# nicolapiccinelli/libmpc

Hardware: AMD Instinct MI355X
Metric: MPC solves/sec (whole node) + p50 solve latency, quadrotor LMPC N=20 batch=4096 (higher is better)
Workload: dtype f64; 1 GPU; quadrotor_ex.cpp LMPC nx=12 nu=4 ny=12 ph=ch=20, batch 4096 per GPU, SplitMix64 x0/u0/yref (SURVEY 8d), maximum_iteration=250; parallelism=single GPU, rccl_ranks=0, streams=1

## Files before the change

### libmpc_amd/csrc/lmpc_fast.hip

```cpp
#include "lmpc_kernel_common.hpp"
#include <cstddef>
#include <cstdlib>

namespace mpcx {

namespace {

#ifndef MPCX_FAST_PF_MAXCAP
#define MPCX_FAST_PF_MAXCAP 12
#endif
#ifndef MPCX_FAST_RB
#define MPCX_FAST_RB 4
#endif
#ifndef MPCX_FAST_PF
#define MPCX_FAST_PF 4
#endif
constexpr int kFastCap = 16;
#ifndef MPCX_FAST_ADD_THETA_LATE
#define MPCX_FAST_ADD_THETA_LATE 0.02
#endif
#ifndef MPCX_FAST_SAFE_AFTER
#define MPCX_FAST_SAFE_AFTER 12
#endif

template <int CTRL>
__device__ __forceinline__ double dpp_mov_d(double v)
{
    int lo = __double2loint(v), hi = __double2hiint(v);
    lo = __builtin_amdgcn_update_dpp(lo, lo, CTRL, 0xF, 0xF, false);
    hi = __builtin_amdgcn_update_dpp(hi, hi, CTRL, 0xF, 0xF, false);
    return __hiloint2double(hi, lo);
}
__device__ __forceinline__ double wave_max_dpp(double v)
{
    v = fmax(v, dpp_mov_d<0xB1>(v));
    v = fmax(v, dpp_mov_d<0x4E>(v));
    v = fmax(v, dpp_mov_d<0x141>(v));
    v = fmax(v, dpp_mov_d<0x140>(v));
    return fmax(fmax(readlane_d(v, 0), readlane_d(v, 16)), fmax(readlane_d(v, 32), readlane_d(v, 48)));
}

#ifdef MPCX_PROFILE_ROUNDS
#define MPCX_LAP(k) do { const long long now_ = (long long)__builtin_readcyclecounter(); pacc[k] += now_ - plast; plast = now_; } while (0)
#define MPCX_LAP_WAIT(k) do { __builtin_amdgcn_s_waitcnt(0); MPCX_LAP(k); } while (0)
#define MPCX_PROF_ARGS , long long (&pacc)[6], long long &plast
#define MPCX_PROF_PASS , pacc, plast
#else
#define MPCX_LAP(k) do {} while (0)
#define MPCX_LAP_WAIT(k) do {} while (0)
#define MPCX_PROF_ARGS
#define MPCX_PROF_PASS
#endif

template <int CAP, int NLO, int CPZ, int CPG>
__device__ __forceinline__ int ws_solve_reg(const gdp gY, const int ldy, const int ldz, const int na, const int lane_in,
                                            const int *wsidx, const double *wsb, const double *t0s, double *lam,
                                            const unsigned (&offz)[CPZ], const unsigned (&offg)[CPG],
                                            double (&wv)[2 * CPZ], double (&gw)[2 * CPG], double &lmax MPCX_PROF_ARGS)
{
    constexpr int PF = CAP > MPCX_FAST_PF_MAXCAP ? 0 : (CAP < MPCX_FAST_PF ? CAP : MPCX_FAST_PF);
    int lane = lane_in;
    asm volatile("" : "+v"(lane));
    const bool real = lane < na;
    const int li = real ? lane : 0;
    const int qi = wsidx[li];
    int qc[CAP];
#pragma unroll
    for (int c = 0; c < CAP; ++c) qc[c] = __builtin_amdgcn_readfirstlane(wsidx[(c < NLO || c < na) ? c : 0]);
    double Sr[CAP];
    const unsigned rowoff = (unsigned)(qi * ldy) * 8u;
    const char MPCX_GAS *const gYb = reinterpret_cast<const char MPCX_GAS *>(gY);
    auto y_at = [&](unsigned off) { return *reinterpret_cast<gdp>(gYb + off); };
    auto row_ld2 = [&](int q, unsigned off) { return *reinterpret_cast<const d2 MPCX_GAS *>(gYb + (unsigned)(q * ldy) * 8u + off); };
#pragma unroll
    for (int c = 0; c < CAP; ++c) Sr[c] = y_at(rowoff + (unsigned)qc[c] * 8u);
    const double dg = y_at(rowoff + (unsigned)qi * 8u);
    d2 pz[PF > 0 ? PF : 1][CPZ], pg[PF > 0 ? PF : 1][CPG];
#pragma unroll
    for (int u = 0; u < PF; ++u) {
#pragma unroll
        for (int c = 0; c < CPZ; ++c) pz[u][c] = row_ld2(qc[u], offz[c]);
#pragma unroll
        for (int c = 0; c < CPG; ++c) pg[u][c] = row_ld2(qc[u], offg[c]);
    }
    double y = real ? t0s[qi < ldz ? qi : qi - ldz + 128 * CPZ] - wsb[li] : 0.0;
    MPCX_LAP_WAIT(1);
    if (!real) {
#pragma unroll
        for (int c = 0; c < CAP; ++c) Sr[c] = 0.0;
    }
#pragma unroll
    for (int c = NLO; c < CAP; ++c) if (c >= na) Sr[c] = lane == c ? 1.0 : 0.0;
    const double pthr = 1e-11 * (real ? dg : 1.0);
    double mydinv = 1.0;
    unsigned long long dep = 0ull;
#pragma unroll
    for (int k = 0; k < CAP; ++k) {
        dep |= __ballot(!(Sr[k] > pthr)) & (1ull << k);
        const double rinv = pivot_rcp(readlane_d(Sr[k], k));
        double pj[CAP];
#pragma unroll
        for (int j = k + 1; j < CAP; ++j) pj[j] = readlane_d(Sr[j], k);
        const double py = readlane_d(y, k);
        if (lane == k) mydinv = rinv;
        else {
            const double m = Sr[k] * rinv;
#pragma unroll
            for (int j = k + 1; j < CAP; ++j) Sr[j] = fma(-m, pj[j], Sr[j]);
            y = fma(-m, py, y);
        }
    }
    MPCX_LAP(2);
    if (dep != 0ull) return (int)__builtin_ctzll(dep);
    y *= mydinv;
    if (real) lam[lane] = y;
#pragma unroll
    for (int c = 0; c < CPZ; ++c) {
        const double2 v = *reinterpret_cast<const double2 *>(t0s + 128 * c + 2 * lane);
        wv[2 * c] = v.x; wv[2 * c + 1] = v.y;
    }
#pragma unroll
    for (int c = 0; c < CPG; ++c) {
        const double2 v = *reinterpret_cast<const double2 *>(t0s + 128 * CPZ + 128 * c + 2 * lane);
        gw[2 * c] = v.x; gw[2 * c + 1] = v.y;
    }
    double lm = 0.0;
#pragma unroll
    for (int a = 0; a < PF; ++a) {
        const double la = readlane_d(y, a);
        lm = fmax(lm, fabs(la));
#pragma unroll
        for (int c = 0; c < CPZ; ++c) { wv[2 * c] = fma(-la, pz[a][c].x, wv[2 * c]); wv[2 * c + 1] = fma(-la, pz[a][c].y, wv[2 * c + 1]); }
#pragma unroll
        for (int c = 0; c < CPG; ++c) { gw[2 * c] = fma(-la, pg[a][c].x, gw[2 * c]); gw[2 * c + 1] = fma(-la, pg[a][c].y, gw[2 * c + 1]); }
    }
    if constexpr (CAP > PF) {
        constexpr int RB = CAP - PF < MPCX_FAST_RB ? CAP - PF : MPCX_FAST_RB;
        int again = 0;
        asm volatile("" : "+s"(again));
        const int *wsidx_again = wsidx + again;
#pragma unroll
        for (int a0 = PF; a0 < CAP; a0 += RB) {
            if (a0 < na) {
                d2 mz[RB][CPZ], mgv[RB][CPG];
#pragma unroll
                for (int u = 0; u < RB; ++u) {
                    const int cu = a0 + u < CAP ? a0 + u : 0;
                    const int q = __builtin_amdgcn_readfirstlane(wsidx_again[(cu < NLO || cu < na) ? cu : 0]);
#pragma unroll
                    for (int c = 0; c < CPZ; ++c) mz[u][c] = row_ld2(q, offz[c]);
#pragma unroll
                    for (int c = 0; c < CPG; ++c) mgv[u][c] = row_ld2(q, offg[c]);
                }
#pragma unroll
                for (int u = 0; u < RB; ++u) {
                    if (a0 + u < CAP) {
                        const double la = readlane_d(y, a0 + u < CAP ? a0 + u : 0);
                        lm = fmax(lm, fabs(la));
#pragma unroll
                        for (int c = 0; c < CPZ; ++c) { wv[2 * c] = fma(-la, mz[u][c].x, wv[2 * c]); wv[2 * c + 1] = fma(-la, mz[u][c].y, wv[2 * c + 1]); }
#pragma unroll
                        for (int c = 0; c < CPG; ++c) { gw[2 * c] = fma(-la, mgv[u][c].x, gw[2 * c]); gw[2 * c + 1] = fma(-la, mgv[u][c].y, gw[2 * c + 1]); }
                    }
                }
            }
        }
    }
    lmax = lm;
    return -1;
}

template <int CPZ, int CPG>
__device__ __forceinline__ void fast_init_pads(double *slice, const int ldz, const int ldg, const int lane)
{
    constexpr int ZP = 128 * CPZ, GPD = 128 * CPG;
    const double INF = __builtin_huge_val();
    double *t0s = slice, *gt0s = t0s + ZP, *lgs = gt0s + GPD, *ugs = lgs + GPD, *fs = ugs + GPD, *lam = fs + ZP + 2;
#pragma unroll
    for (int c = 0; c < CPZ; ++c) {
        const int e = 128 * c + 2 * lane;
        if (e >= ldz) { *reinterpret_cast<double2 *>(t0s + e) = make_double2(0.0, 0.0); *reinterpret_cast<double2 *>(fs + e) = make_double2(0.0, 0.0); }
    }
#pragma unroll
    for (int c = 0; c < CPG; ++c) {
        const int r = 128 * c + 2 * lane;
        if (r >= ldg) {
            *reinterpret_cast<double2 *>(gt0s + r) = make_double2(0.0, 0.0);
            *reinterpret_cast<double2 *>(lgs + r) = make_double2(-INF, -INF);
            *reinterpret_cast<double2 *>(ugs + r) = make_double2(INF, INF);
        }
    }
    if (lane == 0) { lam[kFastCap] = 0.0; lam[kFastCap + 1] = 0.0; }
}

template <int CPZ, int CPG> constexpr int fast_slice_fixed() { return 2 * 128 * CPZ + 3 * 128 * CPG + 2 + 2 * (kFastCap + 2) + (kFastCap + 2) / 2 + 1; }

constexpr int kCpFused = 3;
struct RecPtrs { double *f, *t0, *gt0, *lg, *ug, *tail; };
__device__ __forceinline__ void fused_record(const LmpcDev &M, const LmpcBatchDev &Bt, const int b, const int lane, double *stage,
                                             const RecPtrs &rp, const double *mf_lds)
{
    const int nx = M.nx, nu = M.nu, ny = M.ny, kin = M.kin;
    const int ldz = M.ldz, ldg = M.ldg, ldy = M.ldy, rowsF = M.rowsF;
    const int variant = Bt.fused - 1;
    for (int k = lane; k < kin; k += 64) {
        double v = 0.0;
        if (k < M.nxp) { if (k < nx) v = gl(Bt.x0)[(size_t)b * nx + k]; }
        else if (k < M.nxp + M.nup) { const int c = k - M.nxp; if (c < nu) v = gl(Bt.u0)[(size_t)b * nu + c]; }
        else if (k < M.ione) { const int c = k - M.nxp - M.nup; if (variant && c < ny) v = gl(Bt.yref)[(size_t)b * Bt.yref_bs + c]; }
        else if (k == M.ione) v = 1.0;
        stage[k] = v;
    }
    wave_sync();
    double acc[2 * kCpFused];
#pragma unroll
    for (int s = 0; s < 2 * kCpFused; ++s) acc[s] = 0.0;
    if (mf_lds) {
        int off[kCpFused];
#pragma unroll
        for (int c = 0; c < kCpFused; ++c) { const int e = 128 * c + 2 * lane; off[c] = e < rowsF ? e : 0; }
        for (int j = 0; j < kin; j += 4) {
            double2 m[4][kCpFused];
            double xj[4];
#pragma unroll
            for (int u = 0; u < 4; ++u) {
                const double *col = mf_lds + (size_t)(j + u) * rowsF;
#pragma unroll
                for (int c = 0; c < kCpFused; ++c) m[u][c] = *reinterpret_cast<const double2 *>(col + off[c]);
                xj[u] = stage[j + u];
            }
#pragma unroll
            for (int u = 0; u < 4; ++u) {
#pragma unroll
                for (int c = 0; c < kCpFused; ++c) {
                    acc[2 * c] = fma(m[u][c].x, xj[u], acc[2 * c]);
                    acc[2 * c + 1] = fma(m[u][c].y, xj[u], acc[2 * c + 1]);
                }
            }
        }
    } else {
        matvec_acc<kCpFused>(gl(variant ? M.MF1 : M.MF0), rowsF, rowsF, kin, stage, acc, lane);
    }
    const int r_goff = ldy, r_f = r_goff + ldg, r_s = r_f + ldz, r_q = r_s + M.nsp;
    double c0p = 0.0;
    bool bad = false;
#pragma unroll
    for (int c = 0; c < kCpFused; ++c) {
        const int e = 128 * c + 2 * lane;
        if (e >= rowsF) continue;
        const double a0 = acc[2 * c], a1 = acc[2 * c + 1];
        if (e < ldz) {
            *reinterpret_cast<double2 *>(rp.t0 + e) = make_double2(a0, a1);
        } else if (e < r_goff) {
            *reinterpret_cast<double2 *>(rp.gt0 + (e - ldz)) = make_double2(a0, a1);
        } else if (e < r_f) {
            const int r = e - r_goff;
            const d2 l0 = ld2(GP(lg0) + r), u0 = ld2(GP(ug0) + r);
            *reinterpret_cast<double2 *>(rp.lg + r) = make_double2(l0.x - a0, l0.y - a1);
            *reinterpret_cast<double2 *>(rp.ug + r) = make_double2(u0.x - a0, u0.y - a1);
        } else if (e < r_s) {
            *reinterpret_cast<double2 *>(rp.f + (e - r_f)) = make_double2(a0, a1);
        } else if (e < r_q) {
            const int r = e - r_s;
            if (r < M.ns) bad |= violates(a0, GP(slo)[r], GP(shi)[r], M.eps_abs, M.eps_rel);
            if (r + 1 < M.ns) bad |= violates(a1, GP(slo)[r + 1], GP(shi)[r + 1], M.eps_abs, M.eps_rel);
        } else {
            const int k = e - r_q;
            c0p = fma(0.5 * stage[k], a0, c0p);
            c0p = fma(0.5 * stage[k + 1], a1, c0p);
        }
    }
    c0p = wave_sum(c0p);
    const bool anybad = wave_any(bad);
    if (lane == 0) *reinterpret_cast<double2 *>(rp.tail) = make_double2(c0p, anybad ? 1.0 : 0.0);
    wave_sync();
}

struct GroupArgs { LmpcDev M; LmpcBatchDev Bt; double *wsbase; int variant; };
typedef const GroupArgs __attribute__((address_space(4))) *group_args_p;
static_assert(offsetof(GroupArgs, Bt) == sizeof(LmpcDev) && offsetof(GroupArgs, wsbase) == sizeof(LmpcDev) + sizeof(LmpcBatchDev), "GroupArgs mirrors lmpc_solve_group's parameter list");

template <int CPZ, int CPG, int SRC>
__device__ __forceinline__ void fast_finish(const LmpcDev &M, const LmpcBatchDev &Bt, const int b, const int lane, double *slice, const double *lwuw, gdw ws, double *outs,
                                            const bool infeasible, const bool solved, const bool fixed_violation,
                                            const double (&wv)[2 * CPZ], const int (&actb)[2 * CPZ], const int (&actg)[2 * CPG], const int (&posb)[2 * CPZ],
                                            const int (&posg)[2 * CPG], const double dtol_last, const int na_last, const int rounds_total,
                                            const long long ts0, const long long ts1, const long long ts2 MPCX_PROF_ARGS)
{
    constexpr int NZS = 2 * CPZ, NGS = 2 * CPG, ZP = 128 * CPZ, GPD = 128 * CPG;
    constexpr bool FUSED = SRC != 0;
    const int nx = M.nx, nu = M.nu, ny = M.ny, ndu = M.ndu, ph = M.ph;
    const int nz = M.nz, mg = M.mg, ldz = M.ldz, ldg = M.ldg, ldy = M.ldy;
    double *t0s = slice, *gt0s = t0s + ZP, *lgs = gt0s + GPD, *ugs = lgs + GPD, *fs = ugs + GPD, *tail = fs + ZP;
    double *lam = tail + 2, *wsb = lam + (kFastCap + 2);
    double *scratch = wsb + (kFastCap + 2) + (kFastCap + 2) / 2 + 1;
    const double *lws = lwuw, *uws = lwuw + ZP;
    const double c0 = tail[0], flag0 = tail[1];
    long long ts3 = 0;
    auto stamp = [&](long long &t) { if (Bt.dbg_cycles) t = (long long)__builtin_readcyclecounter(); };

    if (!infeasible && !solved) {
        if constexpr (FUSED) {
#pragma unroll
            for (int c = 0; c < CPZ; ++c) {
                const int e = 128 * c + 2 * lane;
                if (e < ldz) {
                    const double2 vf = *reinterpret_cast<const double2 *>(fs + e), vt = *reinterpret_cast<const double2 *>(t0s + e);
                    st2(ws + e, vf.x, vf.y); st2(ws + ldz + e, vt.x, vt.y);
                }
            }
#pragma unroll
            for (int c = 0; c < CPG; ++c) {
                const int r = 128 * c + 2 * lane;
                if (r < ldg) {
                    const double2 vt = *reinterpret_cast<const double2 *>(gt0s + r), vl = *reinterpret_cast<const double2 *>(lgs + r),
                                  vu = *reinterpret_cast<const double2 *>(ugs + r);
                    st2(ws + ldz + ldz + r, vt.x, vt.y);
                    st2(ws + ldz + ldy + r, vl.x, vl.y);
// ... 75 lines not shown
        unsigned *bl = reinterpret_cast<unsigned *>(t0s);
        unsigned *bu = bl + M.active_words;
        for (int wd = lane; wd < 2 * M.active_words; wd += 64) bl[wd] = 0u;
        wave_sync();
        if (!infeasible) {
#pragma unroll
            for (int s = 0; s < NZS; ++s) {
                const int e = 128 * (s >> 1) + 2 * lane + (s & 1);
                if (e >= nz || actb[s] == 0) continue;
                const double l = lam[posb[s]];
                if (!(fabs(l) > dtol_last)) continue;
                const int side = l < 0 ? -1 : 1;
                const double lo = lws[e], hi = uws[e];
                for (int p = GP(boxrow_ptr)[e]; p < GP(boxrow_ptr)[e + 1]; ++p) {
                    const int rr = GP(boxrow_ref)[p];
                    if (side < 0 && GP(boxrow_lo)[p] == lo) atomicOr(&bl[rr >> 5], 1u << (rr & 31));
                    if (side > 0 && GP(boxrow_hi)[p] == hi) atomicOr(&bu[rr >> 5], 1u << (rr & 31));
                }
            }
#pragma unroll
            for (int s = 0; s < NGS; ++s) {
                const int r = 128 * (s >> 1) + 2 * lane + (s & 1);
                if (r >= mg || actg[s] == 0) continue;
                const double l = lam[posg[s]];
                if (!(fabs(l) > dtol_last)) continue;
                const int rr = GP(g_refrow)[r];
                if (l < 0) atomicOr(&bl[rr >> 5], 1u << (rr & 31));
                else atomicOr(&bu[rr >> 5], 1u << (rr & 31));
            }
        }
        wave_sync();
        for (int wd = lane; wd < M.active_words; wd += 64) {
            glw(Bt.active_lower)[(size_t)b * M.active_words + wd] = bl[wd];
            glw(Bt.active_upper)[(size_t)b * M.active_words + wd] = bu[wd];
        }
        wave_sync();
    }

    if (Bt.seq_state || Bt.seq_input || Bt.seq_output) {
        wave_sync();
        const gdp gA = GP(A), gB = GP(B), gC = GP(C), gBd = GP(Bd), gDd = GP(Dd), gdm = gl(Bt.dmeas ? Bt.dmeas : M.dmeas_s);
        const gip gblk = GP(blk);
        auto dm = [&](int k, int dd) -> double { return ref_at(gdm, Bt.dmeas_bs, Bt.dmeas_ks, b, k, dd); };
        double *xs0 = scratch, *xs1 = scratch + nx;
        if (lane < nx) xs0[lane] = infeasible ? qnan : gl(Bt.x0)[(size_t)b * nx + lane];
        wave_sync();
        for (int i = 0; i <= ph; ++i) {
            const double *xc = (i & 1) ? xs1 : xs0;
            double *xn = (i & 1) ? xs0 : xs1;
            const int k = i > 0 ? i - 1 : 0;
            if (Bt.seq_state && lane < nx) glw(Bt.seq_state)[((size_t)b * (ph + 1) + i) * nx + lane] = xc[lane];
            if (Bt.seq_input && lane < nu) {
                const int ii = (i + 1 <= ph) ? i + 1 : ph;
                glw(Bt.seq_input)[((size_t)b * (ph + 1) + i) * nu + lane] = stage[gblk[ii] * nu + lane];
            }
            if (Bt.seq_output && lane < ny) {
                double yv = 0;
                for (int c = 0; c < nx; ++c) yv = fma(gC[lane + c * ny], xc[c], yv);
                if (M.has_dist) for (int dd = 0; dd < ndu; ++dd) yv = fma(gDd[lane + dd * ny], dm(k, dd), yv);
                glw(Bt.seq_output)[((size_t)b * (ph + 1) + i) * ny + lane] = yv;
            }
            if (i < ph && lane < nx) {
                double s = 0;
                for (int c = 0; c < nx; ++c) s = fma(gA[lane + c * nx], xc[c], s);
                for (int c = 0; c < nu; ++c) s = fma(gB[lane + c * nx], stage[gblk[i + 1] * nu + c], s);
                if (M.has_dist) for (int dd = 0; dd < ndu; ++dd) s = fma(gBd[lane + dd * nx], dm(i, dd), s);
                xn[lane] = s;
            }
            wave_sync();
        }
    }
    wave_sync();
    if (lane == 0 && !outs) ws[ldz + ldy + 2 * ldg + 1] = cost_pending ? 3.0 : 2.0;
    stamp(ts3);
    if (Bt.dbg_cycles && lane == 0)
    {
        long long *o = Bt.dbg_cycles + (size_t)b * 8;
#ifdef MPCX_PROFILE_ROUNDS
        o[0] = ts1 - ts0; o[1] = ts2 - ts1;
        for (int k = 0; k < 6; ++k) o[2 + k] = pacc[k];
#else
        o[0] = ts0; o[1] = ts1; o[2] = ts2; o[3] = ts3;
#endif
    }
}

template <int CPZ, int CPG, int SRC = 0>
__device__ __forceinline__ void solve_fast(const LmpcDev &M, const LmpcBatchDev &Bt, const int b, const int lane,
                           double *slice, const double *lwuw, gdw ws, const double *mf_lds = nullptr, double *outs = nullptr, const int eqbits = 0)
{
    constexpr int NZS = 2 * CPZ, NGS = 2 * CPG, ZP = 128 * CPZ, GPD = 128 * CPG;
    const int nz = M.nz, mg = M.mg, ldz = M.ldz, ldg = M.ldg, ldy = M.ldy;
    const gdp gY = GP(Y);
    double *t0s = slice, *gt0s = t0s + ZP, *lgs = gt0s + GPD, *ugs = lgs + GPD, *fs = ugs + GPD, *tail = fs + ZP;
    double *lam = tail + 2, *wsb = lam + (kFastCap + 2);
    int *wsidx = reinterpret_cast<int *>(wsb + (kFastCap + 2));
    double *scratch = wsb + (kFastCap + 2) + (kFastCap + 2) / 2 + 1;
    const double *lws = lwuw, *uws = lwuw + ZP;
    const double INF = __builtin_huge_val();

    long long ts0 = 0, ts1 = 0, ts2 = 0;
#ifdef MPCX_PROFILE_ROUNDS
    long long pacc[6] = {0, 0, 0, 0, 0, 0}, plast = 0;
#endif
    auto stamp = [&](long long &t) { if (Bt.dbg_cycles) t = (long long)__builtin_readcyclecounter(); };
    stamp(ts0);

    int offz[CPZ], offg[CPG];
#pragma unroll
    for (int c = 0; c < CPZ; ++c) { const int e = 128 * c + 2 * lane; offz[c] = e < ldz ? e : 0; }
#pragma unroll
    for (int c = 0; c < CPG; ++c) { const int r = 128 * c + 2 * lane; offg[c] = ldz + (r < ldg ? r : 0); }
    unsigned boffz[CPZ], boffg[CPG];
#pragma unroll
    for (int c = 0; c < CPZ; ++c) boffz[c] = (unsigned)offz[c] * 8u;
#pragma unroll
    for (int c = 0; c < CPG; ++c) boffg[c] = (unsigned)offg[c] * 8u;

    if constexpr (SRC != 2) fast_init_pads<CPZ, CPG>(slice, ldz, ldg, lane);
    if constexpr (SRC == 2) {
    } else if constexpr (SRC == 1) {
        RecPtrs rp{fs, t0s, gt0s, lgs, ugs, tail};
        fused_record(M, Bt, b, lane, scratch, rp, mf_lds);
    } else {
#pragma unroll
        for (int c = 0; c < CPZ; ++c) {
            const int e = 128 * c + 2 * lane;
            if (e < ldz) {
                const d2 vf = ld2(ws + e), vt = ld2(ws + ldz + e);
                *reinterpret_cast<double2 *>(fs + e) = make_double2(vf.x, vf.y);
                *reinterpret_cast<double2 *>(t0s + e) = make_double2(vt.x, vt.y);
            }
        }
#pragma unroll
        for (int c = 0; c < CPG; ++c) {
            const int r = 128 * c + 2 * lane;
            if (r < ldg) {
                const d2 vt = ld2(ws + 2 * ldz + r), vl = ld2(ws + ldz + ldy + r), vu = ld2(ws + ldz + ldy + ldg + r);
                *reinterpret_cast<double2 *>(gt0s + r) = make_double2(vt.x, vt.y);
                *reinterpret_cast<double2 *>(lgs + r) = make_double2(vl.x, vl.y);
                *reinterpret_cast<double2 *>(ugs + r) = make_double2(vu.x, vu.y);
            }
        }
        if (lane == 0) { const d2 t = ld2(ws + ldz + ldy + 2 * ldg); *reinterpret_cast<double2 *>(tail) = make_double2(t.x, t.y); }
        wave_sync();
    }
    const double flag0 = tail[1];
    const bool fixed_violation = flag0 == 1.0;
    const bool infeasible = fixed_violation && M.strict_infeasible;

    int actb[NZS], actg[NGS];
    const double ptol = 1e-8;
    auto viol = [&](double v, double lo, double hi) {
        return fmax(fmax(lo - ptol * fmax(1.0, fabs(lo)) - v, v - hi - ptol * fmax(1.0, fabs(hi))), 0.0);
    };
    {
        double vb[NZS], vg[NGS], vinit = 0.0;
        bool lowb[NZS], lowg[NGS];
#pragma unroll
        for (int c = 0; c < CPZ; ++c) {
            const int e = 128 * c + 2 * lane;
            const double2 l = *reinterpret_cast<const double2 *>(lws + e), u = *reinterpret_cast<const double2 *>(uws + e);
            const double2 t = *reinterpret_cast<const double2 *>(t0s + e);
            vb[2 * c] = viol(t.x, l.x, u.x); vb[2 * c + 1] = viol(t.y, l.y, u.y);
            lowb[2 * c] = t.x < l.x; lowb[2 * c + 1] = t.y < l.y;
            actb[2 * c] = l.x == u.x ? 2 : 0; actb[2 * c + 1] = l.y == u.y ? 2 : 0;
            vinit = fmax(vinit, fmax(vb[2 * c], vb[2 * c + 1]));
        }
#pragma unroll
        for (int c = 0; c < CPG; ++c) {
            const int r = 128 * c + 2 * lane;
            const double2 l = *reinterpret_cast<const double2 *>(lgs + r), u = *reinterpret_cast<const double2 *>(ugs + r);
            const double2 t = *reinterpret_cast<const double2 *>(gt0s + r);
            vg[2 * c] = viol(t.x, l.x, u.x); vg[2 * c + 1] = viol(t.y, l.y, u.y);
            lowg[2 * c] = t.x < l.x; lowg[2 * c + 1] = t.y < l.y;
            if constexpr (SRC == 2) {
                actg[2 * c] = ((eqbits >> (2 * c)) & 1) ? 2 : 0; actg[2 * c + 1] = ((eqbits >> (2 * c + 1)) & 1) ? 2 : 0;
            } else {
                const d2 l0 = ld2(GP(lg0) + (offg[c] - ldz)), u0 = ld2(GP(ug0) + (offg[c] - ldz));
                const bool ok = r < ldg;
                actg[2 * c] = (ok && l0.x == u0.x) ? 2 : 0; actg[2 * c + 1] = (ok && l0.y == u0.y) ? 2 : 0;
            }
            vinit = fmax(vinit, fmax(vg[2 * c], vg[2 * c + 1]));
        }
        const double thr0 = MPCX_INIT_THETA * wave_max_dpp(vinit);
#pragma unroll
        for (int s = 0; s < NZS; ++s) actb[s] = (actb[s] == 0 && vb[s] > 0.0 && vb[s] >= thr0) ? (lowb[s] ? -1 : 1) : actb[s];
#pragma unroll
        for (int s = 0; s < NGS; ++s) actg[s] = (actg[s] == 0 && vg[s] > 0.0 && vg[s] >= thr0) ? (lowg[s] ? -1 : 1) : actg[s];
    }
    stamp(ts1);

    if (Bt.warm_lower) {
        const unsigned MPCX_GAS *wl = gl(Bt.warm_lower) + (size_t)b * M.active_words;
        const unsigned MPCX_GAS *wu = gl(Bt.warm_upper) + (size_t)b * M.active_words;
        const int na = M.nx + M.nu, n1 = M.ph + 1;
        const int b_box = M.neq_ref, b_out = b_box + n1 * na, b_du = b_out + n1 * M.ny, b_sc = b_du + M.ph * M.nu;
        auto look = [&](int rr) {
            if (!Bt.warm_shift) return rr;
            if (rr < b_out) return rr + na < b_out ? rr + na : rr;
            if (rr < b_du) return rr + M.ny < b_du ? rr + M.ny : rr;
            if (rr < b_sc) return rr;
            return rr + 1 < M.m_ref ? rr + 1 : rr;
        };
#pragma unroll
        for (int s = 0; s < NZS; ++s) {
            const int e = 128 * (s >> 1) + 2 * lane + (s & 1);
            if (e >= nz || actb[s] == 2) continue;
            const double lo = lws[e], hi = uws[e];
            int side = 0;
            for (int p = GP(boxrow_ptr)[e]; p < GP(boxrow_ptr)[e + 1]; ++p) {
                const int rr = look(GP(boxrow_ref)[p]);
                if (((wl[rr >> 5] >> (rr & 31)) & 1u) && GP(boxrow_lo)[p] == lo) side = -1;
                if (((wu[rr >> 5] >> (rr & 31)) & 1u) && GP(boxrow_hi)[p] == hi) side = 1;
            }
            actb[s] = side;
        }
#pragma unroll
        for (int s = 0; s < NGS; ++s) {
            const int r = 128 * (s >> 1) + 2 * lane + (s & 1);
            if (r >= mg || actg[s] == 2) continue;
            const int rr = look(GP(g_refrow)[r]);
            actg[s] = ((wl[rr >> 5] >> (rr & 31)) & 1u) ? -1 : (((wu[rr >> 5] >> (rr & 31)) & 1u) ? 1 : 0);
        }
    }

    double wv[NZS], gw[NGS];
    int posb[NZS], posg[NGS];
    double dtol_last = 0;
    int na_last = 0, rounds_total = 0;
    bool solved = false;

    if (!infeasible && M.polish) {
        const int rounds = M.polish_rounds0;
        for (int rd = 0; rd < rounds; ++rd) {
            ++rounds_total;
#ifdef MPCX_PROFILE_ROUNDS
            plast = (long long)__builtin_readcyclecounter();
#endif
            if (rd == 3) __builtin_amdgcn_s_setprio(1);
            else if (rd == 5) __builtin_amdgcn_s_setprio(2);
            else if (rd == 7) __builtin_amdgcn_s_setprio(3);
            int na = 0;
#pragma unroll
            for (int c = 0; c < CPZ; ++c) {
                const int e = 128 * c + 2 * lane;
                const double2 l = *reinterpret_cast<const double2 *>(lws + e), u = *reinterpret_cast<const double2 *>(uws + e);
#pragma unroll
                for (int h = 0; h < 2; ++h) {
                    const int s = 2 * c + h;
                    const bool act = actb[s] != 0;
                    const unsigned long long mk = __ballot(act);
                    int pos = (int)__builtin_amdgcn_mbcnt_hi((unsigned)(mk >> 32), __builtin_amdgcn_mbcnt_lo((unsigned)mk, (unsigned)na));
                    pos = (act && pos < kFastCap) ? pos : kFastCap;
                    posb[s] = pos;
                    wsidx[pos] = e + h;
                    wsb[pos] = actb[s] < 0 ? (h ? l.y : l.x) : (h ? u.y : u.x);
                    na += __popcll(mk);
                }
            }
#pragma unroll
            for (int c = 0; c < CPG; ++c) {
                const int r = 128 * c + 2 * lane;
                const double2 l = *reinterpret_cast<const double2 *>(lgs + r), u = *reinterpret_cast<const double2 *>(ugs + r);
#pragma unroll
                for (int h = 0; h < 2; ++h) {
                    const int s = 2 * c + h;
                    const bool act = actg[s] != 0;
                    const unsigned long long mk = __ballot(act);
                    int pos = (int)__builtin_amdgcn_mbcnt_hi((unsigned)(mk >> 32), __builtin_amdgcn_mbcnt_lo((unsigned)mk, (unsigned)na));
                    pos = (act && pos < kFastCap) ? pos : kFastCap;
                    posg[s] = pos;
                    wsidx[pos] = ldz + r + h;
                    wsb[pos] = actg[s] < 0 ? (h ? l.y : l.x) : (h ? u.y : u.x);
                    na += __popcll(mk);
                }
            }
            if (na > kFastCap) break;
            na_last = na;
            wave_sync();
            MPCX_LAP_WAIT(0);
            int dep_at = -1;
            double lmax = 0.0;
            if (na == 0) {
#pragma unroll
                for (int c = 0; c < CPZ; ++c) { const double2 v = *reinterpret_cast<const double2 *>(t0s + 128 * c + 2 * lane); wv[2 * c] = v.x; wv[2 * c + 1] = v.y; }
#pragma unroll
                for (int c = 0; c < CPG; ++c) { const double2 v = *reinterpret_cast<const double2 *>(gt0s + 128 * c + 2 * lane); gw[2 * c] = v.x; gw[2 * c + 1] = v.y; }
            } else if (na <= 4) dep_at = ws_solve_reg<4, 1, CPZ, CPG>(gY, ldy, ldz, na, lane, wsidx, wsb, t0s, lam, boffz, boffg, wv, gw, lmax MPCX_PROF_PASS);
            else if (na <= 6) dep_at = ws_solve_reg<6, 5, CPZ, CPG>(gY, ldy, ldz, na, lane, wsidx, wsb, t0s, lam, boffz, boffg, wv, gw, lmax MPCX_PROF_PASS);
            else if (na <= 8) dep_at = ws_solve_reg<8, 7, CPZ, CPG>(gY, ldy, ldz, na, lane, wsidx, wsb, t0s, lam, boffz, boffg, wv, gw, lmax MPCX_PROF_PASS);
            else if (na <= 10) dep_at = ws_solve_reg<10, 9, CPZ, CPG>(gY, ldy, ldz, na, lane, wsidx, wsb, t0s, lam, boffz, boffg, wv, gw, lmax MPCX_PROF_PASS);
            else if (na <= 12) dep_at = ws_solve_reg<12, 11, CPZ, CPG>(gY, ldy, ldz, na, lane, wsidx, wsb, t0s, lam, boffz, boffg, wv, gw, lmax MPCX_PROF_PASS);
            else if (na <= 14) dep_at = ws_solve_reg<14, 13, CPZ, CPG>(gY, ldy, ldz, na, lane, wsidx, wsb, t0s, lam, boffz, boffg, wv, gw, lmax MPCX_PROF_PASS);
            else dep_at = ws_solve_reg<kFastCap, 15, CPZ, CPG>(gY, ldy, ldz, na, lane, wsidx, wsb, t0s, lam, boffz, boffg, wv, gw, lmax MPCX_PROF_PASS);
            if (dep_at >= 0) {
                const int q = wsidx[dep_at];
#pragma unroll
                for (int s = 0; s < NZS; ++s)
                    if (128 * (s >> 1) + 2 * lane + (s & 1) == q) actb[s] = 0;
#pragma unroll
                for (int s = 0; s < NGS; ++s)
                    if (ldz + 128 * (s >> 1) + 2 * lane + (s & 1) == q) actg[s] = 0;
                wave_sync();
                continue;
            }
            wave_sync();
            MPCX_LAP_WAIT(3);
            const double dtol = 1e-9 * lmax + 1e-300;
            dtol_last = dtol;
            double badb[NZS], badg[NGS], vb[NZS], vg[NGS], vm = 0.0, bm = 0.0, chk = 0.0;
            bool lowb[NZS], lowg[NGS];
            double lmb[NZS], lmg[NGS];
#pragma unroll
            for (int s = 0; s < NZS; ++s) lmb[s] = lam[posb[s]];
#pragma unroll
            for (int s = 0; s < NGS; ++s) lmg[s] = lam[posg[s]];
#pragma unroll
            for (int c = 0; c < CPZ; ++c) {
                const int e = 128 * c + 2 * lane;
                const double2 l = *reinterpret_cast<const double2 *>(lws + e), u = *reinterpret_cast<const double2 *>(uws + e);
#pragma unroll
                for (int h = 0; h < 2; ++h) {
                    const int s = 2 * c + h;
                    const double lo = h ? l.y : l.x, hi = h ? u.y : u.x;
                    chk += wv[s];
                    lowb[s] = wv[s] < lo;
                    const double v = viol(wv[s], lo, hi);
                    vb[s] = actb[s] == 0 ? v : 0.0;
                    badb[s] = actb[s] == -1 ? lmb[s] : (actb[s] == 1 ? -lmb[s] : 0.0);
                    vm = fmax(vm, vb[s]); bm = fmax(bm, badb[s]);
                }
            }
#pragma unroll
            for (int c = 0; c < CPG; ++c) {
                const int r = 128 * c + 2 * lane;
                const double2 l = *reinterpret_cast<const double2 *>(lgs + r), u = *reinterpret_cast<const double2 *>(ugs + r);
#pragma unroll
                for (int h = 0; h < 2; ++h) {
                    const int s = 2 * c + h;
                    const double lo = h ? l.y : l.x, hi = h ? u.y : u.x;
                    chk += gw[s];
                    lowg[s] = gw[s] < lo;
                    const double v = viol(gw[s], lo, hi);
                    vg[s] = actg[s] == 0 ? v : 0.0;
                    badg[s] = actg[s] == -1 ? lmg[s] : (actg[s] == 1 ? -lmg[s] : 0.0);
                    vm = fmax(vm, vg[s]); bm = fmax(bm, badg[s]);
                }
            }
            if (wave_any(!(chk - chk == 0.0))) break;
            MPCX_LAP(4);
            const bool any_bad = wave_any(bm > dtol), any_viol = wave_any(vm > 0.0);
            if (!any_bad && !any_viol) { solved = true; break; }
            if (rd < MPCX_FAST_SAFE_AFTER) {
                const double thr = any_viol ? (rd < 3 ? MPCX_FAST_ADD_THETA : MPCX_FAST_ADD_THETA_LATE) * wave_max_dpp(vm) : INF;
#pragma unroll
                for (int s = 0; s < NZS; ++s) actb[s] = badb[s] > dtol ? 0 : ((vb[s] > 0.0 && vb[s] >= thr) ? (lowb[s] ? -1 : 1) : actb[s]);
#pragma unroll
                for (int s = 0; s < NGS; ++s) actg[s] = badg[s] > dtol ? 0 : ((vg[s] > 0.0 && vg[s] >= thr) ? (lowg[s] ? -1 : 1) : actg[s]);
            } else {
                const double mx = wave_max_dpp(any_bad ? bm : vm);
                int slot = -1;
#pragma unroll
                for (int s = 0; s < NZS; ++s) if (slot < 0 && (any_bad ? badb[s] : vb[s]) == mx) slot = s;
#pragma unroll
                for (int s = 0; s < NGS; ++s) if (slot < 0 && (any_bad ? badg[s] : vg[s]) == mx) slot = NZS + s;
                const unsigned long long mk = __ballot(slot >= 0);
                if (slot >= 0 && lane == (int)__builtin_ctzll(mk)) {
#pragma unroll
                    for (int s = 0; s < NZS; ++s) if (slot == s) actb[s] = any_bad ? 0 : (lowb[s] ? -1 : 1);
#pragma unroll
                    for (int s = 0; s < NGS; ++s) if (slot == NZS + s) actg[s] = any_bad ? 0 : (lowg[s] ? -1 : 1);
                }
            }
            wave_sync();
            MPCX_LAP(5);
        }
    }
    __builtin_amdgcn_s_setprio(0);
    stamp(ts2);

    if constexpr (SRC == 2) {
        group_args_p ka = (group_args_p)__builtin_amdgcn_kernarg_segment_ptr();
        asm volatile("" : "+s"(ka));
        fast_finish<CPZ, CPG, SRC>((const LmpcDev &)ka->M, (const LmpcBatchDev &)ka->Bt, b, lane, slice, lwuw, ws, outs, infeasible, solved, fixed_violation,
                                   wv, actb, actg, posb, posg, dtol_last, na_last, rounds_total, ts0, ts1, ts2 MPCX_PROF_PASS);
    } else {
        fast_finish<CPZ, CPG, SRC>(M, Bt, b, lane, slice, lwuw, ws, outs, infeasible, solved, fixed_violation,
                                   wv, actb, actg, posb, posg, dtol_last, na_last, rounds_total, ts0, ts1, ts2 MPCX_PROF_PASS);
    }
}

#ifndef MPCX_FAST_WAVES1
#define MPCX_FAST_WAVES1 4
#endif
#ifndef MPCX_FAST_WAVES2
#define MPCX_FAST_WAVES2 2
#endif
template <int CPZ> constexpr int fast_waves() { return CPZ == 1 ? MPCX_FAST_WAVES1 : (CPZ == 2 ? MPCX_FAST_WAVES2 : 2); }

template <int CPZ>
__device__ __forceinline__ void fast_load_box(const LmpcDev &M, double *lwuw)
{
    constexpr int ZP = 128 * CPZ;
    const double INF = __builtin_huge_val();
    for (int e = 2 * (int)threadIdx.x; e < ZP; e += 2 * (int)blockDim.x) {
        const bool ok = e < M.ldz;
        const d2 vl = ld2(GP(lw) + (ok ? e : 0)), vu = ld2(GP(uw) + (ok ? e : 0));
        *reinterpret_cast<double2 *>(lwuw + e) = ok ? make_double2(vl.x, vl.y) : make_double2(-INF, -INF);
        *reinterpret_cast<double2 *>(lwuw + ZP + e) = ok ? make_double2(vu.x, vu.y) : make_double2(INF, INF);
    }
    __syncthreads();
}

template <int CPZ, int CPG>
__global__ __launch_bounds__(kWavesPerBlock * 64, fast_waves<CPZ>()) void lmpc_solve(const LmpcDev *__restrict__ Mp, const LmpcBatchDev Bt, double *wsbase)
{
    extern __shared__ __attribute__((aligned(16))) double smem[];
    const LmpcDev &M = *Mp;
    const int lane = threadIdx.x & 63, wave = threadIdx.x >> 6;
    constexpr int ZP = 128 * CPZ;
    const int wpb = blockDim.x >> 6;
    double *rec = smem + 2 * ZP + (size_t)wave * M.fast_slice;
    fast_load_box<CPZ>(M, smem);
    const int i = blockIdx.x * wpb + wave;
    if (i < Bt.batch) solve_fast<CPZ, CPG, 0>(M, Bt, i, lane, rec, smem, glw(wsbase) + (size_t)i * M.wsld);
}

template <int CPZ, int CPG>
__global__ __launch_bounds__(kWavesPerBlock * 64, fast_waves<CPZ>()) void lmpc_solve_hetero(const LmpcDev *__restrict__ Mp, const LmpcBatchDev Bt, double *wsbase)
{
    extern __shared__ __attribute__((aligned(16))) double smem[];
    const LmpcDev &M = *Mp;
    const int lane = threadIdx.x & 63, wave = threadIdx.x >> 6;
    constexpr int ZP = 128 * CPZ;
    const int wpb = blockDim.x >> 6;
    double *rec = smem + 2 * ZP + (size_t)wave * M.fast_slice;
    double *box = smem + 2 * ZP + (size_t)wpb * M.fast_slice + (size_t)wave * 2 * ZP;
    const double INF = __builtin_huge_val();
    const int i = blockIdx.x * wpb + wave;
    if (i < Bt.batch) {
        const LmpcDev &Mi = Mp[lmpc_model_of(Bt, i)];
#pragma unroll
        for (int c = 0; c < CPZ; ++c) {
            const int e = 128 * c + 2 * lane;
            const bool ok = e < Mi.ldz;
            const d2 vl = ld2(gl(Mi.lw) + (ok ? e : 0)), vu = ld2(gl(Mi.uw) + (ok ? e : 0));
            *reinterpret_cast<double2 *>(box + e) = ok ? make_double2(vl.x, vl.y) : make_double2(-INF, -INF);
            *reinterpret_cast<double2 *>(box + ZP + e) = ok ? make_double2(vu.x, vu.y) : make_double2(INF, INF);
        }
        wave_sync();
        solve_fast<CPZ, CPG, 0>(Mi, Bt, i, lane, rec, box, glw(wsbase) + (size_t)i * M.wsld);
        wave_sync();
    }
}

template <int CPZ, int CPG>
__global__ __launch_bounds__(kWavesPerBlock * 64, fast_waves<CPZ>()) void lmpc_solve_fused(const LmpcDev *__restrict__ Mp, const LmpcBatchDev Bt, double *wsbase)
{
    extern __shared__ __attribute__((aligned(16))) double smem[];
    const LmpcDev &M = *Mp;
    const int lane = threadIdx.x & 63, wave = threadIdx.x >> 6;
    fast_load_box<CPZ>(M, smem);
    double *rec = smem + 2 * 128 * CPZ + (size_t)wave * M.fast_slice;
    const int wpb = blockDim.x >> 6;
    const int b = blockIdx.x * wpb + wave;
    if (b < Bt.batch) solve_fast<CPZ, CPG, 1>(M, Bt, b, lane, rec, smem, glw(wsbase) + (size_t)b * M.wsld);
}

constexpr int kPersistWaves = 12;
template <int CPZ, int CPG>
__global__ __launch_bounds__(kPersistWaves * 64) void lmpc_solve_persistent(const LmpcDev *__restrict__ Mp, const LmpcBatchDev Bt, double *wsbase,
                                                                             int *counter)
{
    extern __shared__ __attribute__((aligned(16))) double smem[];
    const LmpcDev &M = *Mp;
    const int lane = threadIdx.x & 63, wave = threadIdx.x >> 6;
    const int nmf = M.rowsF * M.kin;
    {
        const gdp src = gl(Bt.fused == 2 ? M.MF1 : M.MF0);
        for (int k = 2 * (int)threadIdx.x; k < nmf; k += 2 * (int)blockDim.x) {
            const d2 v = ld2(src + k);
            *reinterpret_cast<double2 *>(smem + k) = make_double2(v.x, v.y);
        }
    }
    double *lwuw = smem + nmf;
    fast_load_box<CPZ>(M, lwuw);
    double *rec = lwuw + 2 * 128 * CPZ + (size_t)wave * M.fast_slice;
    const int nwaves = gridDim.x * kPersistWaves, shard = blockIdx.x & 7;
    int b = blockIdx.x * kPersistWaves + wave;
    while (b < Bt.batch) {
        solve_fast<CPZ, CPG, 1>(M, Bt, b, lane, rec, lwuw, glw(wsbase) + (size_t)b * M.wsld, smem);
        int n = 0;
        if (lane == 0) n = atomicAdd(counter + shard, 1);
        n = __builtin_amdgcn_readfirstlane(n);
        b = nwaves + shard + 8 * n;
    }
}

template <size_t BYTES>
__device__ __forceinline__ void kernarg_touch()
{
    static_assert(BYTES <= 16 * 64 && BYTES > 15 * 64, "kernarg_touch covers sixteen lines, the sixteenth must exist");
    const auto ka = __builtin_amdgcn_kernarg_segment_ptr();
    int t0, t1, t2, t3, t4, t5, t6, t7, t8, t9, t10, t11, t12, t13, t14, t15;
    asm volatile("s_load_dword %0, %16, 0x0\n\ts_load_dword %1, %16, 0x40\n\ts_load_dword %2, %16, 0x80\n\ts_load_dword %3, %16, 0xc0\n\t"
                 "s_load_dword %4, %16, 0x100\n\ts_load_dword %5, %16, 0x140\n\ts_load_dword %6, %16, 0x180\n\ts_load_dword %7, %16, 0x1c0\n\t"
                 "s_load_dword %8, %16, 0x200\n\ts_load_dword %9, %16, 0x240\n\ts_load_dword %10, %16, 0x280\n\ts_load_dword %11, %16, 0x2c0\n\t"
                 "s_load_dword %12, %16, 0x300\n\ts_load_dword %13, %16, 0x340\n\ts_load_dword %14, %16, 0x380\n\ts_load_dword %15, %16, 0x3c0\n\t"
                 "s_waitcnt lgkmcnt(0)"
                 : "=&s"(t0), "=&s"(t1), "=&s"(t2), "=&s"(t3), "=&s"(t4), "=&s"(t5), "=&s"(t6), "=&s"(t7), "=&s"(t8), "=&s"(t9), "=&s"(t10), "=&s"(t11),
                   "=&s"(t12), "=&s"(t13), "=&s"(t14), "=&s"(t15)
                 : "s"(ka)
                 : "memory");
}
#ifndef MPCX_GROUP_BALANCE
#define MPCX_GROUP_BALANCE 1
#endif

template <int CPZ> constexpr int kGroupWavesOf = CPZ == 1 ? 16 : 8;
constexpr int kGroupG2 = 5;
constexpr int kGroupG1 = 2;
template <int CPZ, int CPG>
__global__ __launch_bounds__(kGroupWavesOf<CPZ> * 64) void lmpc_solve_group(const LmpcDev Mv, const LmpcBatchDev Btv, double *wsbasev, const int variantv)
{
    constexpr int kGroupWaves = kGroupWavesOf<CPZ>;
    extern __shared__ __attribute__((aligned(16))) double smem[];
#if defined(MPCX_GROUP_CUT) && MPCX_GROUP_CUT == 0
    { return; }
#endif
    kernarg_touch<sizeof(LmpcDev) + sizeof(LmpcBatchDev) + sizeof(double *) + sizeof(int)>();
    const group_args_p ka = (group_args_p)__builtin_amdgcn_kernarg_segment_ptr();
    const LmpcDev &M = (const LmpcDev &)ka->M;
    const LmpcBatchDev &Bt = (const LmpcBatchDev &)ka->Bt;
    double *const wsbase = ka->wsbase;
    const int variant = ka->variant;
    const int lane = threadIdx.x & 63, wave = threadIdx.x >> 6;
    const int j = lane & 15, kq = lane >> 4;
    const int nx = M.nx, nu = M.nu, ny = M.ny;
    const int kin4 = M.kin >> 2, nz4 = M.nz16 >> 2;
    const int ldz = M.ldz, ldg = M.ldg, ldy = M.ldy;
    constexpr int ZP = 128 * CPZ, GPD = 128 * CPG;
    double *lwuw = smem;
    double *slices = lwuw + 2 * ZP;
    double *Bv = slices + (size_t)kGroupWaves * M.fast_slice;
    double *Bf = Bv + (size_t)kin4 * 64;
    double *c0s = Bf + (size_t)nz4 * 64;
    unsigned *bad = reinterpret_cast<unsigned *>(c0s + kGroupWaves * 16);
    const int outld = 8 + ((nu + 1) & ~1);
    double *outs = c0s + kGroupWaves * 16 + 16;
    double *mine = slices + (size_t)wave * M.fast_slice;
    const gdp MAp = gl(variant ? M.MA1p : M.MA0p), Ymp = GP(Ymp);
    const int ntile1 = M.rowsA >> 4, tg = M.nz16 >> 4, ts = tg + (M.mg16 >> 4), tq = ts + (M.ns16 >> 4);
    const int ntile2 = M.ldy16 >> 4;
    const int G1 = (kin4 + 3) >> 2, G2 = (nz4 + 3) >> 2;
    auto ld4 = [](gdp p) -> v4d { return *reinterpret_cast<const v4d MPCX_GAS *>(p); };
    const bool jlive = j < kGroupWaves;
    double *sj = slices + (size_t)(jlive ? j : 0) * M.fast_slice;
    double *t0j = sj, *gt0j = sj + ZP, *lgj = gt0j + GPD, *ugj = lgj + GPD, *fj = ugj + GPD;

    const int b0 = blockIdx.x * kGroupWaves;
    const int bj = b0 + (jlive ? j : kGroupWaves - 1);
    const int bc = bj < Bt.batch ? bj : Bt.batch - 1;
    auto gstamp = [&](int k) { if (Bt.dbg_cycles && lane == 0 && b0 + wave < Bt.batch) Bt.dbg_cycles[(size_t)(b0 + wave) * 8 + k] = (long long)__builtin_readcyclecounter(); };
    gstamp(4);

    auto vin_at = [&](int kb) -> double {
        const int k = 4 * kb + kq;
        gdp src = gl(Bt.x0);
        bool ld = false;
        if (k < M.nxp) { ld = k < nx; src = gl(Bt.x0) + ((size_t)bc * nx + k); }
        else if (k < M.nxp + M.nup) { const int c = k - M.nxp; ld = c < nu; src = gl(Bt.u0) + ((size_t)bc * nu + c); }
        else if (k < M.ione) { const int c = k - M.nxp - M.nup; ld = variant && c < ny; src = gl(Bt.yref) + ((size_t)bc * Bt.yref_bs + c); }
        double v = k == M.ione ? 1.0 : 0.0;
        if (ld) v = *src;
        return v;
    };
    const double vin0 = wave < kin4 ? vin_at(wave) : 0.0;
    const int ebx = 2 * (int)threadIdx.x;
    const bool boxok = ebx < ldz;
    d2 bxl = {0.0, 0.0}, bxu = {0.0, 0.0};
    if (ebx < ZP) { bxl = ld2(GP(lw) + (boxok ? ebx : 0)); bxu = ld2(GP(uw) + (boxok ? ebx : 0)); }
    const int t1 = wave < ntile1 ? wave : ntile1 - 1;
    v4d a1[kGroupG1];
#pragma unroll
    for (int g = 0; g < kGroupG1; ++g) a1[g] = ld4(MAp + (((size_t)t1 * G1 + (g < G1 ? g : 0)) * 64 + lane) * 4);
    double eblo[4], ebhi[4];
    {
        const bool ing = t1 >= tg && t1 < ts, ins = t1 >= ts && t1 < tq;
        const gdp plo = ing ? GP(lg0) + 16 * (t1 - tg) : GP(slo) + 16 * (ins ? t1 - ts : 0);
        const gdp phi = ing ? GP(ug0) + 16 * (t1 - tg) : GP(shi) + 16 * (ins ? t1 - ts : 0);
        const int lim = ing ? ldg - 16 * (t1 - tg) : (ins ? M.ns - 16 * (t1 - ts) : 0);
#pragma unroll
        for (int r = 0; r < 4; ++r) {
            const int row = 4 * r + kq;
            eblo[r] = 0.0; ebhi[r] = 0.0;
            if (row < lim) { eblo[r] = plo[row]; ebhi[r] = phi[row]; }
        }
    }
    const int t2 = wave < ntile2 ? wave : ntile2 - 1;
    v4d a2[kGroupG2];
#pragma unroll
    for (int g = 0; g < kGroupG2; ++g) a2[g] = ld4(Ymp + (((size_t)t2 * G2 + (g < G2 ? g : 0)) * 64 + lane) * 4);
    d2 eql[CPG], equ[CPG];
#pragma unroll
    for (int c = 0; c < CPG; ++c) {
        const int r = 128 * c + 2 * lane;
        eql[c] = d2{0.0, 0.0}; equ[c] = d2{1.0, 1.0};
        if (wave == kGroupWaves - 1) { eql[c] = ld2(GP(lg0) + (r < ldg ? r : 0)); equ[c] = ld2(GP(ug0) + (r < ldg ? r : 0)); }
    }

    fast_init_pads<CPZ, CPG>(mine, ldz, ldg, lane);
    if (wave < kin4) Bv[wave * 64 + lane] = vin0;
    for (int kb = wave + kGroupWaves; kb < kin4; kb += kGroupWaves) Bv[kb * 64 + lane] = vin_at(kb);
    if (ebx < ZP) {
        const double INF = __builtin_huge_val();
        *reinterpret_cast<double2 *>(lwuw + ebx) = boxok ? make_double2(bxl.x, bxl.y) : make_double2(-INF, -INF);
        *reinterpret_cast<double2 *>(lwuw + ZP + ebx) = boxok ? make_double2(bxu.x, bxu.y) : make_double2(INF, INF);
    }
    if (threadIdx.x < 16) bad[threadIdx.x] = 0u;
    __syncthreads();
    gstamp(7);
#if defined(MPCX_GROUP_CUT) && MPCX_GROUP_CUT == 1
    { return; }
#endif

    {
        double c0p = 0.0;
        bool badl = false;
        auto tile1 = [&]<bool PRE>(const int t) {
// ... 261 lines not shown
```

Before: 120.6 million solves/s.

## Multi-buffer working-set row loads and tighten wave reductions and sign checks

After: 124.7 million solves/s (median of 6 runs). +3.4%, better.

```diff
diff --git a/libmpc_amd/csrc/lmpc_fast.hip b/libmpc_amd/csrc/lmpc_fast.hip
--- a/libmpc_amd/csrc/lmpc_fast.hip
+++ b/libmpc_amd/csrc/lmpc_fast.hip
@@ -15,6 +15,21 @@
 #ifndef MPCX_FAST_PF
 #define MPCX_FAST_PF 4
 #endif
+#ifndef MPCX_FAST_PF_ALL
+#define MPCX_FAST_PF_ALL 6
+#endif
+#ifndef MPCX_FAST_NBUF
+#define MPCX_FAST_NBUF 3
+#endif
+#ifndef MPCX_FAST_RB_DEEP
+#define MPCX_FAST_RB_DEEP 2
+#endif
+#ifndef MPCX_FAST_DEEP_CHUNKS
+#define MPCX_FAST_DEEP_CHUNKS 4
+#endif
+#ifndef MPCX_FAST_STAGE
+#define MPCX_FAST_STAGE() __builtin_amdgcn_sched_barrier(0)
+#endif
 constexpr int kFastCap = 16;
 #ifndef MPCX_FAST_ADD_THETA_LATE
 #define MPCX_FAST_ADD_THETA_LATE 0.02
@@ -26,9 +41,8 @@
 template <int CTRL>
 __device__ __forceinline__ double dpp_mov_d(double v)
 {
-    int lo = __double2loint(v), hi = __double2hiint(v);
-    lo = __builtin_amdgcn_update_dpp(lo, lo, CTRL, 0xF, 0xF, false);
-    hi = __builtin_amdgcn_update_dpp(hi, hi, CTRL, 0xF, 0xF, false);
+    const int lo = __builtin_amdgcn_mov_dpp(__double2loint(v), CTRL, 0xF, 0xF, true);
+    const int hi = __builtin_amdgcn_mov_dpp(__double2hiint(v), CTRL, 0xF, 0xF, true);
     return __hiloint2double(hi, lo);
 }
 __device__ __forceinline__ double wave_max_dpp(double v)
@@ -37,7 +51,9 @@
     v = fmax(v, dpp_mov_d<0x4E>(v));
     v = fmax(v, dpp_mov_d<0x141>(v));
     v = fmax(v, dpp_mov_d<0x140>(v));
-    return fmax(fmax(readlane_d(v, 0), readlane_d(v, 16)), fmax(readlane_d(v, 32), readlane_d(v, 48)));
+    v = fmax(v, dpp_mov_d<0x142>(v));
+    v = fmax(v, dpp_mov_d<0x143>(v));
+    return readlane_d(v, 63);
 }
 
 #ifdef MPCX_PROFILE_ROUNDS
@@ -58,7 +74,8 @@
                                             const unsigned (&offz)[CPZ], const unsigned (&offg)[CPG],
                                             double (&wv)[2 * CPZ], double (&gw)[2 * CPG], double &lmax MPCX_PROF_ARGS)
 {
-    constexpr int PF = CAP > MPCX_FAST_PF_MAXCAP ? 0 : (CAP < MPCX_FAST_PF ? CAP : MPCX_FAST_PF);
+    constexpr bool DEEP = CPZ + CPG <= MPCX_FAST_DEEP_CHUNKS;
+    constexpr int PF = CAP > MPCX_FAST_PF_MAXCAP ? 0 : (CAP <= (DEEP ? MPCX_FAST_PF_ALL : MPCX_FAST_PF) ? CAP : MPCX_FAST_PF);
     int lane = lane_in;
     asm volatile("" : "+v"(lane));
     const bool real = lane < na;
@@ -125,45 +142,47 @@
         gw[2 * c] = v.x; gw[2 * c + 1] = v.y;
     }
     double lm = 0.0;
-#pragma unroll
-    for (int a = 0; a < PF; ++a) {
+    auto apply_row = [&](const int a, const d2 (&rz)[CPZ], const d2 (&rg)[CPG]) {
         const double la = readlane_d(y, a);
         lm = fmax(lm, fabs(la));
 #pragma unroll
-        for (int c = 0; c < CPZ; ++c) { wv[2 * c] = fma(-la, pz[a][c].x, wv[2 * c]); wv[2 * c + 1] = fma(-la, pz[a][c].y, wv[2 * c + 1]); }
-#pragma unroll
-        for (int c = 0; c < CPG; ++c) { gw[2 * c] = fma(-la, pg[a][c].x, gw[2 * c]); gw[2 * c + 1] = fma(-la, pg[a][c].y, gw[2 * c + 1]); }
-    }
-    if constexpr (CAP > PF) {
-        constexpr int RB = CAP - PF < MPCX_FAST_RB ? CAP - PF : MPCX_FAST_RB;
+        for (int c = 0; c < CPZ; ++c) { wv[2 * c] = fma(-la, rz[c].x, wv[2 * c]); wv[2 * c + 1] = fma(-la, rz[c].y, wv[2 * c + 1]); }
+#pragma unroll
+        for (int c = 0; c < CPG; ++c) { gw[2 * c] = fma(-la, rg[c].x, gw[2 * c]); gw[2 * c + 1] = fma(-la, rg[c].y, gw[2 * c + 1]); }
+    };
+    if constexpr (CAP == PF) {
+#pragma unroll
+        for (int a = 0; a < PF; ++a) apply_row(a, pz[a], pg[a]);
+    } else {
+        constexpr int RB0 = DEEP ? MPCX_FAST_RB_DEEP : MPCX_FAST_RB, RB = CAP - PF < RB0 ? CAP - PF : RB0;
+        constexpr int NB = (CAP - PF + RB - 1) / RB, NBUF = DEEP ? MPCX_FAST_NBUF : 1;
+        static_assert(PF + (NB - 1) * RB < NLO, "a later batch would start past the class's smallest working set");
         int again = 0;
         asm volatile("" : "+s"(again));
         const int *wsidx_again = wsidx + again;
-#pragma unroll
-        for (int a0 = PF; a0 < CAP; a0 += RB) {
-            if (a0 < na) {
-                d2 mz[RB][CPZ], mgv[RB][CPG];
-#pragma unroll
-                for (int u = 0; u < RB; ++u) {
-                    const int cu = a0 + u < CAP ? a0 + u : 0;
-                    const int q = __builtin_amdgcn_readfirstlane(wsidx_again[(cu < NLO || cu < na) ? cu : 0]);
-#pragma unroll
-                    for (int c = 0; c < CPZ; ++c) mz[u][c] = row_ld2(q, offz[c]);
-#pragma unroll
-                    for (int c = 0; c < CPG; ++c) mgv[u][c] = row_ld2(q, offg[c]);
-                }
-#pragma unroll
-                for (int u = 0; u < RB; ++u) {
-                    if (a0 + u < CAP) {
-                        const double la = readlane_d(y, a0 + u < CAP ? a0 + u : 0);
-                        lm = fmax(lm, fabs(la));
-#pragma unroll
-                        for (int c = 0; c < CPZ; ++c) { wv[2 * c] = fma(-la, mz[u][c].x, wv[2 * c]); wv[2 * c + 1] = fma(-la, mz[u][c].y, wv[2 * c + 1]); }
-#pragma unroll
-                        for (int c = 0; c < CPG; ++c) { gw[2 * c] = fma(-la, mgv[u][c].x, gw[2 * c]); gw[2 * c + 1] = fma(-la, mgv[u][c].y, gw[2 * c + 1]); }
-                    }
-                }
-            }
+        d2 mz[NBUF][RB][CPZ], mgv[NBUF][RB][CPG];
+        auto request = [&](const int k, d2 (&bz)[RB][CPZ], d2 (&bg)[RB][CPG]) {
+#pragma unroll
+            for (int u = 0; u < RB; ++u) {
+                const int cu = PF + k * RB + u < CAP ? PF + k * RB + u : 0;
+                const int q = __builtin_amdgcn_readfirstlane(wsidx_again[(cu < NLO || cu < na) ? cu : 0]);
+#pragma unroll
+                for (int c = 0; c < CPZ; ++c) bz[u][c] = row_ld2(q, offz[c]);
+#pragma unroll
+                for (int c = 0; c < CPG; ++c) bg[u][c] = row_ld2(q, offg[c]);
+            }
+        };
+#pragma unroll
+        for (int a = 0; a < PF; ++a) apply_row(a, pz[a], pg[a]);
+#pragma unroll
+        for (int k = 0; k < NBUF && k < NB; ++k) request(k, mz[k], mgv[k]);
+        MPCX_FAST_STAGE();
+#pragma unroll
+        for (int k = 0; k < NB; ++k) {
+#pragma unroll
+            for (int u = 0; u < RB; ++u)
+                if (PF + k * RB + u < CAP) apply_row(PF + k * RB + u, mz[k % NBUF][u], mgv[k % NBUF][u]);
+            if (k + NBUF < NB) { request(k + NBUF, mz[k % NBUF], mgv[k % NBUF]); MPCX_FAST_STAGE(); }
         }
     }
     lmax = lm;
@@ -545,7 +564,13 @@
     int actb[NZS], actg[NGS];
     const double ptol = 1e-8;
     auto viol = [&](double v, double lo, double hi) {
-        return fmax(fmax(lo - ptol * fmax(1.0, fabs(lo)) - v, v - hi - ptol * fmax(1.0, fabs(hi))), 0.0);
+        const double lo_wide = fma(-ptol, fmax(1.0, fabs(lo)), lo), hi_scale = fmax(1.0, fabs(hi));
+        return fmax(fmax(lo_wide - v, fma(-ptol, hi_scale, v - hi)), 0.0);
+    };
+    auto wrong_signed = [](double lm, int act) {
+        const int in = -(act & 1);
+        const int hi = (__double2hiint(lm) ^ (int)((unsigned)(act + 1) << 30)) & in;
+        return __hiloint2double(hi, __double2loint(lm) & in);
     };
     {
         double vb[NZS], vg[NGS], vinit = 0.0;
@@ -721,7 +746,7 @@
                     lowb[s] = wv[s] < lo;
                     const double v = viol(wv[s], lo, hi);
                     vb[s] = actb[s] == 0 ? v : 0.0;
-                    badb[s] = actb[s] == -1 ? lmb[s] : (actb[s] == 1 ? -lmb[s] : 0.0);
+                    badb[s] = wrong_signed(lmb[s], actb[s]);
                     vm = fmax(vm, vb[s]); bm = fmax(bm, badb[s]);
                 }
             }
@@ -737,7 +762,7 @@
                     lowg[s] = gw[s] < lo;
                     const double v = viol(gw[s], lo, hi);
                     vg[s] = actg[s] == 0 ? v : 0.0;
-                    badg[s] = actg[s] == -1 ? lmg[s] : (actg[s] == 1 ? -lmg[s] : 0.0);
+                    badg[s] = wrong_signed(lmg[s], actg[s]);
                     vm = fmax(vm, vg[s]); bm = fmax(bm, badg[s]);
                 }
             }
@@ -811,7 +836,7 @@
 {
     extern __shared__ __attribute__((aligned(16))) double smem[];
     const LmpcDev &M = *Mp;
-    const int lane = threadIdx.x & 63, wave = threadIdx.x >> 6;
+    const int lane = threadIdx.x & 63, wave = __builtin_amdgcn_readfirstlane(threadIdx.x >> 6);
     constexpr int ZP = 128 * CPZ;
     const int wpb = blockDim.x >> 6;
     double *rec = smem + 2 * ZP + (size_t)wave * M.fast_slice;
@@ -825,7 +850,7 @@
 {
     extern __shared__ __attribute__((aligned(16))) double smem[];
     const LmpcDev &M = *Mp;
-    const int lane = threadIdx.x & 63, wave = threadIdx.x >> 6;
+    const int lane = threadIdx.x & 63, wave = __builtin_amdgcn_readfirstlane(threadIdx.x >> 6);
     constexpr int ZP = 128 * CPZ;
     const int wpb = blockDim.x >> 6;
     double *rec = smem + 2 * ZP + (size_t)wave * M.fast_slice;
@@ -853,7 +878,7 @@
 {
     extern __shared__ __attribute__((aligned(16))) double smem[];
     const LmpcDev &M = *Mp;
-    const int lane = threadIdx.x & 63, wave = threadIdx.x >> 6;
+    const int lane = threadIdx.x & 63, wave = __builtin_amdgcn_readfirstlane(threadIdx.x >> 6);
     fast_load_box<CPZ>(M, smem);
     double *rec = smem + 2 * 128 * CPZ + (size_t)wave * M.fast_slice;
     const int wpb = blockDim.x >> 6;
@@ -868,7 +893,7 @@
 {
     extern __shared__ __attribute__((aligned(16))) double smem[];
     const LmpcDev &M = *Mp;
-    const int lane = threadIdx.x & 63, wave = threadIdx.x >> 6;
+    const int lane = threadIdx.x & 63, wave = __builtin_amdgcn_readfirstlane(threadIdx.x >> 6);
     const int nmf = M.rowsF * M.kin;
     {
         const gdp src = gl(Bt.fused == 2 ? M.MF1 : M.MF0);
```
